# nv-tlabs/GEN3C

Hardware: NVIDIA H100
Metric: denoise-steps/sec, 7B DiT, 121-frame 720p latent (higher is better)
Workload: dtype bf16

## Files before the change

gen3c_b200/csrc/gemm_wgmma.cu:

```cuda
#include <cstdlib>
#include <cstring>

#include "kernels.h"

namespace g3c {

constexpr int BM = 128;
constexpr int BK = 64;
constexpr int WG_K = 16;
template <bool kFp8>
constexpr int kBlockK = kFp8 ? 2 * BK : BK;
constexpr int GEMM_THREADS = 384;

struct GemmParams {
  int M, N, K;
  int ldd;
  void* D;
  const float* gate;
  int num_m_blk, num_n_blk, num_k_blk;
  int super_n;
  const float* nr_gamma;
  const float* nr_cs;
  float nr_eps;
  const float* scale_a;
  const float* scale_b;
};

constexpr int EPI_NORM_ROPE_BF16 = 4;

template <int BN>
struct GemmSmem {
  static constexpr int kABytes = BM * BK * 2;
  static constexpr int kBBytes = BN * BK * 2;
  static constexpr int kStageBytes = kABytes + kBBytes;
  static constexpr int kStages = (192 * 1024) / kStageBytes;
  static constexpr int kBarBytes = 256;
  static constexpr int kTotal = kStages * kStageBytes + kBarBytes + 1024;
};

__device__ __forceinline__ float gelu_erf(float x) {
  return 0.5f * x * (1.0f + erff(x * 0.70710678118654752440f));
}

__device__ __forceinline__ void tile_coords(const GemmParams& p, int tile, int& m_blk, int& n_blk) {
  int per_super = p.num_m_blk * p.super_n;
  int sc = tile / per_super;
  int rem = tile - sc * per_super;
  int n0 = sc * p.super_n;
  int width = p.num_n_blk - n0 < p.super_n ? p.num_n_blk - n0 : p.super_n;
  m_blk = rem / width;
  n_blk = n0 + rem - m_blk * width;
}

template <int BN>
__device__ __forceinline__ void epilogue_norm_rope(const float (&acc)[BN / 2], const GemmParams& p, int row_a, int col_q,
                                                   int n_base) {
#pragma unroll
  for (int hd = 0; hd < BN / 128; ++hd) {
    if (n_base + hd * 128 >= p.N) break;
    float ss[2] = {0.f, 0.f};
#pragma unroll
    for (int i = 16 * hd; i < 16 * hd + 16; ++i) {
      ss[0] = fmaf(acc[4 * i], acc[4 * i], fmaf(acc[4 * i + 1], acc[4 * i + 1], ss[0]));
      ss[1] = fmaf(acc[4 * i + 2], acc[4 * i + 2], fmaf(acc[4 * i + 3], acc[4 * i + 3], ss[1]));
    }
#pragma unroll
    for (int h = 0; h < 2; ++h) {
      ss[h] += __shfl_xor_sync(0xffffffffu, ss[h], 1);
      ss[h] += __shfl_xor_sync(0xffffffffu, ss[h], 2);
    }
#pragma unroll
    for (int h = 0; h < 2; ++h) {
      const int row = row_a + 8 * h;
      if (row >= p.M) continue;
      const float rstd = rsqrtf(ss[h] * (1.0f / 128.0f) + p.nr_eps);
      const float* cs = p.nr_cs ? p.nr_cs + (size_t)row * 128 : nullptr;
      __nv_bfloat16* dptr = reinterpret_cast<__nv_bfloat16*>(p.D) + (size_t)row * p.ldd + n_base + hd * 128;
#pragma unroll
      for (int i = 0; i < 8; ++i) {
        const int c = 8 * i + col_q;
        const float2 ga = *reinterpret_cast<const float2*>(p.nr_gamma + c);
        const float2 gb = *reinterpret_cast<const float2*>(p.nr_gamma + 64 + c);
        const int ia = 4 * (16 * hd + i) + 2 * h, ib = 4 * (16 * hd + i + 8) + 2 * h;
        float a[2] = {acc[ia] * (rstd * ga.x), acc[ia + 1] * (rstd * ga.y)};
        float b[2] = {acc[ib] * (rstd * gb.x), acc[ib + 1] * (rstd * gb.y)};
        if (cs) {
          const float2 co = *reinterpret_cast<const float2*>(cs + c);
          const float2 si = *reinterpret_cast<const float2*>(cs + 64 + c);
          const float cv[2] = {co.x, co.y}, sv[2] = {si.x, si.y};
#pragma unroll
          for (int e = 0; e < 2; ++e) {
            const float n = a[e] * cv[e] - b[e] * sv[e], m = b[e] * cv[e] + a[e] * sv[e];
            a[e] = n;
            b[e] = m;
          }
        }
        *reinterpret_cast<uint32_t*>(dptr + c) = pack_bf16x2(a[0], a[1]);
        *reinterpret_cast<uint32_t*>(dptr + 64 + c) = pack_bf16x2(b[0], b[1]);
      }
    }
  }
}

template <int BN>
__device__ __forceinline__ void dequantise(float (&acc)[BN / 2], const GemmParams& p, int row_a, int col_q, int n_base) {
  float sa[2];
#pragma unroll
  for (int h = 0; h < 2; ++h) sa[h] = row_a + 8 * h < p.M ? p.scale_a[row_a + 8 * h] : 0.f;
#pragma unroll
  for (int i = 0; i < BN / 8; ++i) {
    const int col = n_base + 8 * i + col_q;
    float2 sb = make_float2(0.f, 0.f);
    if (col + 1 < p.N) sb = *reinterpret_cast<const float2*>(p.scale_b + col);
    else if (col < p.N) sb.x = p.scale_b[col];
#pragma unroll
    for (int h = 0; h < 2; ++h) {
      acc[4 * i + 2 * h] = acc[4 * i + 2 * h] * sa[h] * sb.x;
      acc[4 * i + 2 * h + 1] = acc[4 * i + 2 * h + 1] * sa[h] * sb.y;
    }
  }
}

template <int BN, int EPI>
__device__ __forceinline__ void epilogue(const float (&acc)[BN / 2], const GemmParams& p, int row_a, int col_q,
                                         int n_base) {
  if constexpr (EPI == EPI_NORM_ROPE_BF16) {
    epilogue_norm_rope<BN>(acc, p, row_a, col_q, n_base);
  } else {
#pragma unroll
    for (int h = 0; h < 2; ++h) {
      const int row = row_a + 8 * h;
      if (row >= p.M) continue;
#pragma unroll
      for (int i = 0; i < BN / 8; ++i) {
        const int col = n_base + 8 * i + col_q;
        if (col >= p.N) continue;
        const bool pair = col + 1 < p.N;
        float v0 = acc[4 * i + 2 * h], v1 = acc[4 * i + 2 * h + 1];
        if constexpr (EPI == G3C_EPI_BF16 || EPI == G3C_EPI_GELU_BF16) {
          if constexpr (EPI == G3C_EPI_GELU_BF16) {
            v0 = gelu_erf(v0);
            v1 = gelu_erf(v1);
          }
          __nv_bfloat16* dptr = reinterpret_cast<__nv_bfloat16*>(p.D) + (size_t)row * p.ldd + col;
          if (pair) *reinterpret_cast<uint32_t*>(dptr) = pack_bf16x2(v0, v1);
          else dptr[0] = __float2bfloat16_rn(v0);
        } else {
          float* dptr = reinterpret_cast<float*>(p.D) + (size_t)row * p.ldd + col;
          if constexpr (EPI == G3C_EPI_GATED_RESIDUAL_F32) {
            if (pair) {
              const float2 g = *reinterpret_cast<const float2*>(p.gate + col);
              float2 x = *reinterpret_cast<float2*>(dptr);
              x.x = fmaf(g.x, v0, x.x);
              x.y = fmaf(g.y, v1, x.y);
              *reinterpret_cast<float2*>(dptr) = x;
            } else {
              dptr[0] = fmaf(p.gate[col], v0, dptr[0]);
            }
          } else {
            if (pair) *reinterpret_cast<float2*>(dptr) = make_float2(v0, v1);
            else dptr[0] = v0;
          }
        }
      }
    }
  }
}

template <int BN, int EPI, bool kFp8>
__global__ void __launch_bounds__(GEMM_THREADS, 1)
    k_gemm(const __grid_constant__ CUtensorMap tmA, const __grid_constant__ CUtensorMap tmB, const GemmParams p) {
  using S = GemmSmem<BN>;
  constexpr int kStages = S::kStages;
  extern __shared__ uint8_t smem_raw[];
  uint8_t* smem = reinterpret_cast<uint8_t*>((reinterpret_cast<uintptr_t>(smem_raw) + 1023) &
                                             ~static_cast<uintptr_t>(1023));
  uint8_t* smem_a = smem;
  uint8_t* smem_b = smem + kStages * S::kABytes;
  uint64_t* bars = reinterpret_cast<uint64_t*>(smem + kStages * S::kStageBytes);
  uint64_t* full = bars;
  uint64_t* empty = bars + kStages;

  const uint32_t wg = threadIdx.x / 128;
  const uint32_t tid = threadIdx.x % 128;

  if (threadIdx.x == 0) {
    tma_prefetch_desc(&tmA);
    tma_prefetch_desc(&tmB);
    for (int i = 0; i < kStages; ++i) {
      mbar_init(&full[i], 1);
      mbar_init(&empty[i], 2);
    }
    fence_barrier_init();
  }
  __syncthreads();

  const int num_tiles = p.num_m_blk * p.num_n_blk;

  if (wg == 0) {
    setmaxnreg_dec<40>();
    if (tid == 0) {
      uint32_t stage = 0, phase = 0;
      for (int tile = blockIdx.x; tile < num_tiles; tile += gridDim.x) {
        int m_blk, n_blk;
        tile_coords(p, tile, m_blk, n_blk);
        for (int kb = 0; kb < p.num_k_blk; ++kb) {
          mbar_wait(&empty[stage], phase ^ 1);
          mbar_expect_tx(&full[stage], S::kStageBytes);
          tma_load_2d(smem_a + stage * S::kABytes, &tmA, &full[stage], kb * kBlockK<kFp8>, m_blk * BM);
          tma_load_2d(smem_b + stage * S::kBBytes, &tmB, &full[stage], kb * kBlockK<kFp8>, n_blk * BN);
          if (++stage == kStages) {
            stage = 0;
            phase ^= 1;
          }
        }
      }
    }
  } else {
    setmaxnreg_inc<232>();
    const uint32_t c = wg - 1;
    const uint32_t warp = tid / 32, lane = tid % 32;
    uint32_t stage = 0, phase = 0;
    float acc[BN / 2];
    for (int tile = blockIdx.x; tile < num_tiles; tile += gridDim.x) {
      int m_blk, n_blk;
      tile_coords(p, tile, m_blk, n_blk);
      if constexpr (kFp8) {
        static_assert(BN <= 128, "fp8 tiles hold two accumulator sets");
        float part[BN / 2];
#pragma unroll
        for (int i = 0; i < BN / 2; ++i) acc[i] = 0.f;
        for (int kb = 0; kb < p.num_k_blk; ++kb) {
          mbar_wait(&full[stage], phase);
          const uint64_t da = make_sdesc_sw128(smem_u32(smem_a + stage * S::kABytes + c * 64 * 128));
          const uint64_t db = make_sdesc_sw128(smem_u32(smem_b + stage * S::kBBytes));
          wgmma_fence();
#pragma unroll
          for (int k = 0; k < BK / WG_K; ++k) {
            const uint64_t a = sdesc_advance(da, k * WG_K * 2), b = sdesc_advance(db, k * WG_K * 2);
            if constexpr (BN == 128) wgmma_ss_n128_e4m3(part, a, b, k != 0 ? 1u : 0u);
            else wgmma_ss_n64_e4m3(part, a, b, k != 0 ? 1u : 0u);
          }
          wgmma_commit();
          wgmma_wait<0>();
          fence_regs(part);
          if (tid == 0) mbar_arrive(&empty[stage]);
#pragma unroll
          for (int i = 0; i < BN / 2; ++i) acc[i] += part[i];
          if (++stage == kStages) {
            stage = 0;
            phase ^= 1;
          }
        }
      } else {
        uint32_t prev_stage = 0;
        for (int kb = 0; kb < p.num_k_blk; ++kb) {
          mbar_wait(&full[stage], phase);
          const uint64_t da = make_sdesc_sw128(smem_u32(smem_a + stage * S::kABytes + c * 64 * 128));
          const uint64_t db = make_sdesc_sw128(smem_u32(smem_b + stage * S::kBBytes));
          wgmma_fence();
#pragma unroll
          for (int k = 0; k < BK / WG_K; ++k) {
            const uint64_t a = sdesc_advance(da, k * WG_K * 2), b = sdesc_advance(db, k * WG_K * 2);
            const uint32_t accumulate = (kb | k) != 0 ? 1u : 0u;
            if constexpr (BN == 256) wgmma_ss_n256(acc, a, b, accumulate);
            else if constexpr (BN == 128) wgmma_ss_n128(acc, a, b, accumulate);
            else wgmma_ss_n64(acc, a, b, accumulate);
          }
          wgmma_commit();
          wgmma_wait<1>();
          fence_regs(acc);
          if (kb > 0 && tid == 0) mbar_arrive(&empty[prev_stage]);
          prev_stage = stage;
          if (++stage == kStages) {
            stage = 0;
            phase ^= 1;
          }
        }
        wgmma_wait<0>();
        fence_regs(acc);
        if (tid == 0) mbar_arrive(&empty[prev_stage]);
      }
      const int row_a = m_blk * BM + (int)(c * 64 + warp * 16 + lane / 4), col_q = (int)(2 * (lane % 4));
      if constexpr (kFp8) dequantise<BN>(acc, p, row_a, col_q, n_blk * BN);
      epilogue<BN, EPI>(acc, p, row_a, col_q, n_blk * BN);
    }
  }
}

template <int BN, int EPI, bool kFp8>
static int launch_gemm(const CUtensorMap& tmA, const CUtensorMap& tmB, const GemmParams& p, cudaStream_t st) {
  using S = GemmSmem<BN>;
  static bool configured = false;
  if (!configured) {
    G3C_CUDA(cudaFuncSetAttribute(k_gemm<BN, EPI, kFp8>, cudaFuncAttributeMaxDynamicSharedMemorySize, S::kTotal));
    configured = true;
  }
  int tiles = p.num_m_blk * p.num_n_blk;
  int grid = tiles < sm_count() ? tiles : sm_count();
  k_gemm<BN, EPI, kFp8><<<grid, GEMM_THREADS, S::kTotal, st>>>(tmA, tmB, p);
  G3C_CUDA(cudaGetLastError());
  return G3C_OK;
}

template <int BN, bool kFp8>
static int dispatch_epi(int epi, const CUtensorMap& tmA, const CUtensorMap& tmB, const GemmParams& p, cudaStream_t st) {
  switch (epi) {
    case G3C_EPI_BF16: return launch_gemm<BN, G3C_EPI_BF16, kFp8>(tmA, tmB, p, st);
    case G3C_EPI_GELU_BF16: return launch_gemm<BN, G3C_EPI_GELU_BF16, kFp8>(tmA, tmB, p, st);
    case G3C_EPI_GATED_RESIDUAL_F32: return launch_gemm<BN, G3C_EPI_GATED_RESIDUAL_F32, kFp8>(tmA, tmB, p, st);
    case G3C_EPI_F32: return launch_gemm<BN, G3C_EPI_F32, kFp8>(tmA, tmB, p, st);
    case EPI_NORM_ROPE_BF16:
      if constexpr (BN >= 128) return launch_gemm<BN, EPI_NORM_ROPE_BF16, kFp8>(tmA, tmB, p, st);
      break;
  }
  set_error("gemm: unknown epilogue %d", epi);
  return G3C_EINVAL;
}

static int gemm_any(const void* A, const void* B, const float* scale_a, const float* scale_b, void* D, int M, int N,
                    int K, int lda, int ldb, int ldd, int epilogue, const float* gate, int block_n, cudaStream_t st,
                    const NormRope* norm_rope) {
  const bool fp8 = scale_a != nullptr;
  G3C_REQUIRE(A && B && D, "gemm: null operand");
  G3C_REQUIRE(epilogue >= G3C_EPI_BF16 && epilogue <= G3C_EPI_F32, "gemm: unknown epilogue %d", epilogue);
  if (norm_rope) {
    G3C_REQUIRE(epilogue == G3C_EPI_BF16 && N % 128 == 0 && norm_rope->gamma,
                "gemm: the RMSNorm/RoPE epilogue needs the bf16 epilogue, N %% 128 == 0 and a gain vector");
    G3C_REQUIRE((reinterpret_cast<uintptr_t>(norm_rope->gamma) & 15) == 0 &&
                    (reinterpret_cast<uintptr_t>(norm_rope->cs) & 15) == 0,
                "gemm: RMSNorm gain / RoPE table must be 16-byte aligned");
    epilogue = EPI_NORM_ROPE_BF16;
  }
  G3C_REQUIRE(M > 0 && N > 0 && K > 0, "gemm: bad shape %dx%dx%d", M, N, K);
  if (fp8)
    G3C_REQUIRE(K % 16 == 0 && lda % 16 == 0 && ldb % 16 == 0, "gemm_fp8: K/lda/ldb must be multiples of 16");
  else
    G3C_REQUIRE(K % 8 == 0 && lda % 8 == 0 && ldb % 8 == 0, "gemm: K/lda/ldb must be multiples of 8");
  G3C_REQUIRE(lda >= K && ldb >= K && ldd >= N, "gemm: leading dimension smaller than extent");
  if (epilogue == G3C_EPI_BF16 || epilogue == G3C_EPI_GELU_BF16 || epilogue == EPI_NORM_ROPE_BF16)
    G3C_REQUIRE(ldd % 8 == 0 && (reinterpret_cast<uintptr_t>(D) & 15) == 0,
                "gemm: bf16 output needs ldd %% 8 == 0 and 16-byte aligned base");
  else
    G3C_REQUIRE(ldd % 4 == 0 && (reinterpret_cast<uintptr_t>(D) & 15) == 0,
                "gemm: f32 output needs ldd %% 4 == 0 and 16-byte aligned base");
  G3C_REQUIRE(epilogue != G3C_EPI_GATED_RESIDUAL_F32 ||
                  (gate && (reinterpret_cast<uintptr_t>(gate) & 15) == 0),
              "gemm: gated-residual epilogue needs a 16-byte aligned gate vector");
  int bn = block_n;
  G3C_REQUIRE(bn == 0 || bn == 64 || bn == 128 || bn == 256 || bn == 512, "gemm: block_n %d unsupported", bn);
  if (bn == 512) {
    G3C_REQUIRE(N % 256 == 0, "gemm: block_n 512 needs N %% 256 == 0 (N=%d)", N);
    bn = 256;
  }
  if (bn == 0) bn = (N >= 256 && N % 256 == 0) ? 256 : (N > 64 ? 128 : 64);
  if (fp8 && bn == 256) bn = 128;
  G3C_REQUIRE(epilogue != EPI_NORM_ROPE_BF16 || bn >= 128, "gemm: the RMSNorm/RoPE epilogue needs tiles of whole heads");

  CUtensorMap tmA, tmB;
  const int esize = fp8 ? 1 : 2, bk = fp8 ? kBlockK<true> : kBlockK<false>;
  const CUtensorMapDataType dt = fp8 ? CU_TENSOR_MAP_DATA_TYPE_UINT8 : CU_TENSOR_MAP_DATA_TYPE_BFLOAT16;
  uint64_t dimsA[2] = {(uint64_t)K, (uint64_t)M}, strA[1] = {(uint64_t)lda * esize};
  uint32_t boxA[2] = {(uint32_t)bk, BM};
  int rc = make_tmap_bf16_sw128(&tmA, A, 2, dimsA, strA, boxA, dt);
  if (rc) return rc;
  uint64_t dimsB[2] = {(uint64_t)K, (uint64_t)N}, strB[1] = {(uint64_t)ldb * esize};
  uint32_t boxB[2] = {(uint32_t)bk, (uint32_t)bn};
  rc = make_tmap_bf16_sw128(&tmB, B, 2, dimsB, strB, boxB, dt);
  if (rc) return rc;

  GemmParams p;
  p.M = M;
  p.N = N;
  p.K = K;
  p.ldd = ldd;
  p.D = D;
  p.gate = gate;
  p.nr_gamma = norm_rope ? norm_rope->gamma : nullptr;
  p.nr_cs = norm_rope ? norm_rope->cs : nullptr;
  p.nr_eps = norm_rope ? norm_rope->eps : 0.0f;
  p.scale_a = scale_a;
  p.scale_b = scale_b;
  p.num_m_blk = (M + BM - 1) / BM;
  p.num_n_blk = (N + bn - 1) / bn;
  p.num_k_blk = (K + bk - 1) / bk;
  long long col_bytes = (long long)bn * K * esize;
  int sn = (int)((16ll << 20) / (col_bytes > 0 ? col_bytes : 1));
  if (sn < 1) sn = 1;
  if (sn > p.num_n_blk) sn = p.num_n_blk;
  p.super_n = sn;
  if (fp8) return bn == 64 ? dispatch_epi<64, true>(epilogue, tmA, tmB, p, st)
                           : dispatch_epi<128, true>(epilogue, tmA, tmB, p, st);
  switch (bn) {
    case 64: return dispatch_epi<64, false>(epilogue, tmA, tmB, p, st);
    case 128: return dispatch_epi<128, false>(epilogue, tmA, tmB, p, st);
    default: return dispatch_epi<256, false>(epilogue, tmA, tmB, p, st);
  }
}

int gemm_bf16(const void* A, const void* B, void* D, int M, int N, int K, int lda, int ldb, int ldd,
              int epilogue, const float* gate, int block_n, cudaStream_t st, const NormRope* norm_rope) {
  return gemm_any(A, B, nullptr, nullptr, D, M, N, K, lda, ldb, ldd, epilogue, gate, block_n, st, norm_rope);
}

int gemm_fp8(const void* A8, const float* scale_a, const void* B8, const float* scale_b, void* D, int M, int N, int K,
             int lda, int ldb, int ldd, int epilogue, const float* gate, int block_n, cudaStream_t st,
             const NormRope* norm_rope) {
  G3C_REQUIRE(scale_a && scale_b, "gemm_fp8: null scale vector");
  G3C_REQUIRE((reinterpret_cast<uintptr_t>(scale_a) & 15) == 0 && (reinterpret_cast<uintptr_t>(scale_b) & 15) == 0,
              "gemm_fp8: scale vectors must be 16-byte aligned");
  return gemm_any(A8, B8, scale_a, scale_b, D, M, N, K, lda, ldb, ldd, epilogue, gate, block_n, st, norm_rope);
}

}

extern "C" int g3c_gemm_bf16(const void* A, const void* B, void* D, int M, int N, int K, int lda,
                             int ldb, int ldd, int epilogue, const float* gate, int block_n,
                             void* stream) {
  return g3c::gemm_bf16(A, B, D, M, N, K, lda, ldb, ldd, epilogue, gate, block_n,
                        (cudaStream_t)stream);
}

extern "C" int g3c_gemm_fp8(const void* A8, const float* scale_A, const void* B8, const float* scale_B, void* D, int M,
                            int N, int K, int lda, int ldb, int ldd, int epilogue, const float* gate, int block_n,
                            void* stream) {
  return g3c::gemm_fp8(A8, scale_A, B8, scale_B, D, M, N, K, lda, ldb, ldd, epilogue, gate, block_n,
                       (cudaStream_t)stream);
}

extern "C" int g3c_gemm_norm_rope_fp8(const void* A8, const float* scale_A, const void* B8, const float* scale_B, void* D,
                                      int M, int N, int K, int lda, int ldb, int ldd, const float* gamma,
                                      const float* cos_sin, float eps, void* stream) {
  g3c::NormRope nr;
  nr.gamma = gamma;
  nr.cs = cos_sin;
  nr.eps = eps;
  return g3c::gemm_fp8(A8, scale_A, B8, scale_B, D, M, N, K, lda, ldb, ldd, G3C_EPI_BF16, nullptr, 0,
                       (cudaStream_t)stream, &nr);
}

extern "C" int g3c_gemm_norm_rope_bf16(const void* A, const void* B, void* D, int M, int N, int K, int lda, int ldb,
                                       int ldd, const float* gamma, const float* cos_sin, float eps, void* stream) {
  g3c::NormRope nr;
  nr.gamma = gamma;
  nr.cs = cos_sin;
  nr.eps = eps;
  return g3c::gemm_bf16(A, B, D, M, N, K, lda, ldb, ldd, G3C_EPI_BF16, nullptr, 0, (cudaStream_t)stream, &nr);
}
```

gen3c_b200/csrc/common.cuh:

```cuda
#pragma once
#include <cuda.h>
#include <cuda_bf16.h>
#include <cuda_runtime.h>
#include <stdint.h>
#include <stdio.h>

#include "../../include/gen3c_b200.h"
#include "wgmma_ops.cuh"

namespace g3c {

void set_error(const char* fmt, ...);
int cuda_fail(cudaError_t e, const char* what, const char* file, int line);
#define G3C_CUDA(x)                                                         \
  do {                                                                      \
    cudaError_t _e = (x);                                                   \
    if (_e != cudaSuccess) return ::g3c::cuda_fail(_e, #x, __FILE__, __LINE__); \
  } while (0)
#define G3C_REQUIRE(cond, ...)        \
  do {                                \
    if (!(cond)) {                    \
      ::g3c::set_error(__VA_ARGS__);  \
      return G3C_EINVAL;       \
    }                                 \
// ... 66 lines not shown
  return ok != 0;
}
__device__ __forceinline__ bool mbar_test(uint64_t* bar, uint32_t parity) {
  uint32_t ok;
  asm volatile(
      "{\n\t.reg .pred P;\n\t"
      "mbarrier.test_wait.parity.shared::cta.b64 P, [%1], %2;\n\t"
      "selp.b32 %0, 1, 0, P;\n\t}\n"
      : "=r"(ok)
      : "r"(smem_u32(bar)), "r"(parity)
      : "memory");
  return ok != 0;
}
#ifndef G3C_MBAR_TIMEOUT_NS
#define G3C_MBAR_TIMEOUT_NS 4000000000ull
#endif
__device__ __forceinline__ uint64_t global_timer_ns() {
  uint64_t t;
  asm volatile("mov.u64 %0, %%globaltimer;\n" : "=l"(t));
  return t;
}
#ifdef G3C_MBAR_DEBUG
#define G3C_MBAR_TIMEOUT_ACTION(bar, parity)                                                                 \
  do {                                                                                                       \
    printf("g3c: mbarrier timeout block(%d,%d) thread %d bar@%u parity %u\n", blockIdx.x, blockIdx.y,        \
           threadIdx.x, bar, parity);                                                                        \
    __trap();                                                                                                \
  } while (0)
#else
#define G3C_MBAR_TIMEOUT_ACTION(bar, parity) asm volatile("trap;\n")
#endif
__device__ __forceinline__ void mbar_wait(uint64_t* bar, uint32_t parity) {
  if (mbar_try_wait(bar, parity)) return;
  uint32_t spins = 0;
  uint64_t t0 = 0;
  while (!mbar_try_wait(bar, parity)) {
    if ((++spins & 0xFFFu) == 0) {
      uint64_t now = global_timer_ns();
      if (t0 == 0) t0 = now;
      else if (now - t0 > G3C_MBAR_TIMEOUT_NS) G3C_MBAR_TIMEOUT_ACTION(smem_u32(bar), parity);
    }
  }
}

__device__ __forceinline__ void mbar_wait_ns(uint64_t* bar, uint32_t parity, unsigned long long timeout_ns) {
  if (mbar_try_wait(bar, parity)) return;
  uint32_t spins = 0;
  uint64_t t0 = 0;
  while (!mbar_try_wait(bar, parity)) {
    if ((++spins & 0xFFFu) == 0) {
      uint64_t now = global_timer_ns();
      if (t0 == 0) t0 = now;
      else if (now - t0 > timeout_ns) G3C_MBAR_TIMEOUT_ACTION(smem_u32(bar), parity);
    }
  }
}

__device__ __forceinline__ void mbar_wait_ns_or_exit(uint64_t* bar, uint32_t parity, unsigned long long timeout_ns) {
  if (mbar_try_wait(bar, parity)) return;
  uint32_t spins = 0;
  uint64_t t0 = 0;
  while (!mbar_try_wait(bar, parity)) {
    if ((++spins & 0xFFFu) == 0) {
      uint64_t now = global_timer_ns();
      if (t0 == 0) t0 = now;
      else if (now - t0 > timeout_ns) asm volatile("exit;\n");
    }
  }
}

__device__ __forceinline__ bool bar_red_or(uint32_t id, uint32_t nthreads, bool pred) {
  uint32_t r;
  asm volatile(
      "{\n\t.reg .pred P, Q;\n\t"
      "setp.ne.u32 P, %1, 0;\n\t"
      "bar.red.or.pred Q, %2, %3, P;\n\t"
      "selp.u32 %0, 1, 0, Q;\n\t}\n"
      : "=r"(r)
      : "r"((uint32_t)pred), "r"(id), "r"(nthreads)
      : "memory");
  return r != 0;
}

__device__ __forceinline__ void tma_prefetch_desc(const CUtensorMap* m) {
  asm volatile("prefetch.tensormap [%0];\n" ::"l"(reinterpret_cast<uint64_t>(m)) : "memory");
}
__device__ __forceinline__ void tma_load_2d(void* smem_dst, const CUtensorMap* m, uint64_t* bar,
                                            int c0, int c1) {
  asm volatile(
      "cp.async.bulk.tensor.2d.shared::cluster.global.mbarrier::complete_tx::bytes"
      " [%0], [%1, {%3, %4}], [%2];\n" ::"r"(smem_u32(smem_dst)),
      "l"(reinterpret_cast<uint64_t>(m)), "r"(smem_u32(bar)), "r"(c0), "r"(c1)
      : "memory");
}
__device__ __forceinline__ void tma_load_3d(void* smem_dst, const CUtensorMap* m, uint64_t* bar,
                                            int c0, int c1, int c2) {
  asm volatile(
      "cp.async.bulk.tensor.3d.shared::cluster.global.mbarrier::complete_tx::bytes"
      " [%0], [%1, {%3, %4, %5}], [%2];\n" ::"r"(smem_u32(smem_dst)),
      "l"(reinterpret_cast<uint64_t>(m)), "r"(smem_u32(bar)), "r"(c0), "r"(c1), "r"(c2)
      : "memory");
}

__device__ __forceinline__ void tma_store_2d(const CUtensorMap* m, const void* smem_src, int c0, int c1) {
  asm volatile("cp.async.bulk.tensor.2d.global.shared::cta.bulk_group [%0, {%2, %3}], [%1];\n" ::"l"(
                   reinterpret_cast<uint64_t>(m)),
               "r"(smem_u32(smem_src)), "r"(c0), "r"(c1)
               : "memory");
}
__device__ __forceinline__ void tma_reduce_add_2d(const CUtensorMap* m, const void* smem_src, int c0, int c1) {
  asm volatile("cp.reduce.async.bulk.tensor.2d.global.shared::cta.add.bulk_group [%0, {%2, %3}], [%1];\n" ::"l"(
                   reinterpret_cast<uint64_t>(m)),
               "r"(smem_u32(smem_src)), "r"(c0), "r"(c1)
               : "memory");
}
__device__ __forceinline__ void tma_store_commit() { asm volatile("cp.async.bulk.commit_group;\n" ::: "memory"); }
template <int N>
__device__ __forceinline__ void tma_store_wait_read() {
  asm volatile("cp.async.bulk.wait_group.read %0;\n" ::"n"(N) : "memory");
}
template <int N>
__device__ __forceinline__ void tma_store_wait_all() {
  asm volatile("cp.async.bulk.wait_group %0;\n" ::"n"(N) : "memory");
}

__device__ __forceinline__ void wgmma_fence() { asm volatile("wgmma.fence.sync.aligned;\n" ::: "memory"); }
__device__ __forceinline__ void wgmma_commit() { asm volatile("wgmma.commit_group.sync.aligned;\n" ::: "memory"); }
template <int N>
__device__ __forceinline__ void wgmma_wait() {
  asm volatile("wgmma.wait_group.sync.aligned %0;\n" ::"n"(N) : "memory");
}
template <int N>
__device__ __forceinline__ void fence_regs(float (&r)[N]) {
#pragma unroll
  for (int i = 0; i < N; ++i) asm volatile("" : "+f"(r[i])::"memory");
}
template <int N>
__device__ __forceinline__ void fence_regs(uint32_t (&r)[N]) {
#pragma unroll
  for (int i = 0; i < N; ++i) asm volatile("" : "+r"(r[i])::"memory");
}

__device__ __forceinline__ uint64_t make_sdesc_sw128(uint32_t smem_addr) {
  uint64_t d = 0;
  d |= static_cast<uint64_t>((smem_addr & 0x3FFFFu) >> 4);
  d |= static_cast<uint64_t>(1) << 16;
  d |= static_cast<uint64_t>(1024u >> 4) << 32;
  d |= static_cast<uint64_t>(1) << 62;
  return d;
}
__device__ __forceinline__ uint64_t make_sdesc_sw128_mn(uint32_t smem_addr, uint32_t mn_block_bytes) {
  uint64_t d = 0;
  d |= static_cast<uint64_t>((smem_addr & 0x3FFFFu) >> 4);
  d |= static_cast<uint64_t>((mn_block_bytes >> 4) & 0x3FFFu) << 16;
  d |= static_cast<uint64_t>(1024u >> 4) << 32;
  d |= static_cast<uint64_t>(1) << 62;
  return d;
}
__device__ __forceinline__ uint64_t sdesc_advance(uint64_t d, uint32_t bytes) {
  return d + static_cast<uint64_t>(bytes >> 4);
}

template <int N>
__device__ __forceinline__ void setmaxnreg_dec() {
  asm volatile("setmaxnreg.dec.sync.aligned.u32 %0;\n" ::"n"(N));
}
// ... 23 lines not shown
```

Before: 0.1410.

## Vectorise GEMM epilogue stores via quad shuffles and batch gated-residual loads

The bf16 and norm+RoPE epilogues now swap packed values across each lane quad with shuffles, so every thread writes one 16-byte store instead of four 4-byte stores. Gamma for norm+RoPE is staged in shared memory and the cos/sin loads are hoisted out of the per-head loop. The gated-residual epilogue issues its gate and residual loads in batches before the FMAs and stores, giving more memory-level parallelism. The cost is extra shuffle instructions and higher register pressure in the epilogue.

```diff
diff --git a/gen3c_b200/csrc/gemm_wgmma.cu b/gen3c_b200/csrc/gemm_wgmma.cu
--- a/gen3c_b200/csrc/gemm_wgmma.cu
+++ b/gen3c_b200/csrc/gemm_wgmma.cu
@@ -35,7 +35,8 @@
   static constexpr int kStageBytes = kABytes + kBBytes;
   static constexpr int kStages = (192 * 1024) / kStageBytes;
   static constexpr int kBarBytes = 256;
-  static constexpr int kTotal = kStages * kStageBytes + kBarBytes + 1024;
+  static constexpr int kGammaBytes = 128 * 4;
+  static constexpr int kTotal = kStages * kStageBytes + kBarBytes + kGammaBytes + 1024;
 };
 
 __device__ __forceinline__ float gelu_erf(float x) {
@@ -52,51 +53,128 @@
   n_blk = n0 + rem - m_blk * width;
 }
 
+__device__ __forceinline__ uint4 quad_gather_bf16x8(const uint32_t (&v)[4]) {
+  const int lane = (int)(threadIdx.x % 32), q = lane % 4;
+  uint32_t w[4] = {0u, 0u, 0u, 0u};
+#pragma unroll
+  for (int r = 0; r < 4; ++r) {
+    const int js = (q + r) & 3, src = (q - r) & 3;
+    const uint32_t send = js == 0 ? v[0] : js == 1 ? v[1] : js == 2 ? v[2] : v[3];
+    const uint32_t got = r == 0 ? send : __shfl_sync(0xffffffffu, send, (lane & ~3) | src);
+#pragma unroll
+    for (int k = 0; k < 4; ++k) w[k] = src == k ? got : w[k];
+  }
+  return make_uint4(w[0], w[1], w[2], w[3]);
+}
+
 template <int BN>
-__device__ __forceinline__ void epilogue_norm_rope(const float (&acc)[BN / 2], const GemmParams& p, int row_a, int col_q,
-                                                   int n_base) {
-#pragma unroll
-  for (int hd = 0; hd < BN / 128; ++hd) {
-    if (n_base + hd * 128 >= p.N) break;
-    float ss[2] = {0.f, 0.f};
+__device__ __forceinline__ void epilogue_norm_rope(const float (&acc)[BN / 2], const GemmParams& p, const float* gamma_s,
+                                                   int row_a, int col_q, int n_base) {
+  constexpr int kHeads = BN / 128;
+  float ss[kHeads][2];
+#pragma unroll
+  for (int hd = 0; hd < kHeads; ++hd) {
+    ss[hd][0] = ss[hd][1] = 0.f;
 #pragma unroll
     for (int i = 16 * hd; i < 16 * hd + 16; ++i) {
-      ss[0] = fmaf(acc[4 * i], acc[4 * i], fmaf(acc[4 * i + 1], acc[4 * i + 1], ss[0]));
-      ss[1] = fmaf(acc[4 * i + 2], acc[4 * i + 2], fmaf(acc[4 * i + 3], acc[4 * i + 3], ss[1]));
+      ss[hd][0] = fmaf(acc[4 * i], acc[4 * i], fmaf(acc[4 * i + 1], acc[4 * i + 1], ss[hd][0]));
+      ss[hd][1] = fmaf(acc[4 * i + 2], acc[4 * i + 2], fmaf(acc[4 * i + 3], acc[4 * i + 3], ss[hd][1]));
     }
 #pragma unroll
     for (int h = 0; h < 2; ++h) {
-      ss[h] += __shfl_xor_sync(0xffffffffu, ss[h], 1);
-      ss[h] += __shfl_xor_sync(0xffffffffu, ss[h], 2);
-    }
-#pragma unroll
-    for (int h = 0; h < 2; ++h) {
-      const int row = row_a + 8 * h;
-      if (row >= p.M) continue;
-      const float rstd = rsqrtf(ss[h] * (1.0f / 128.0f) + p.nr_eps);
-      const float* cs = p.nr_cs ? p.nr_cs + (size_t)row * 128 : nullptr;
+      ss[hd][h] += __shfl_xor_sync(0xffffffffu, ss[hd][h], 1);
+      ss[hd][h] += __shfl_xor_sync(0xffffffffu, ss[hd][h], 2);
+    }
+  }
+#pragma unroll
+  for (int h = 0; h < 2; ++h) {
+    const int row = row_a + 8 * h;
+    const bool row_ok = row < p.M;
+    float2 co[8], si[8];
+    if (p.nr_cs && row_ok) {
+      const float* cs = p.nr_cs + (size_t)row * 128;
+#pragma unroll
+      for (int i = 0; i < 8; ++i) {
+        co[i] = *reinterpret_cast<const float2*>(cs + 8 * i + col_q);
+        si[i] = *reinterpret_cast<const float2*>(cs + 64 + 8 * i + col_q);
+      }
+    }
+#pragma unroll
+    for (int hd = 0; hd < kHeads; ++hd) {
+      if (n_base + hd * 128 >= p.N) break;
+      const float rstd = rsqrtf(ss[hd][h] * (1.0f / 128.0f) + p.nr_eps);
       __nv_bfloat16* dptr = reinterpret_cast<__nv_bfloat16*>(p.D) + (size_t)row * p.ldd + n_base + hd * 128;
 #pragma unroll
-      for (int i = 0; i < 8; ++i) {
-        const int c = 8 * i + col_q;
-        const float2 ga = *reinterpret_cast<const float2*>(p.nr_gamma + c);
-        const float2 gb = *reinterpret_cast<const float2*>(p.nr_gamma + 64 + c);
-        const int ia = 4 * (16 * hd + i) + 2 * h, ib = 4 * (16 * hd + i + 8) + 2 * h;
-        float a[2] = {acc[ia] * (rstd * ga.x), acc[ia + 1] * (rstd * ga.y)};
-        float b[2] = {acc[ib] * (rstd * gb.x), acc[ib + 1] * (rstd * gb.y)};
-        if (cs) {
-          const float2 co = *reinterpret_cast<const float2*>(cs + c);
-          const float2 si = *reinterpret_cast<const float2*>(cs + 64 + c);
-          const float cv[2] = {co.x, co.y}, sv[2] = {si.x, si.y};
-#pragma unroll
-          for (int e = 0; e < 2; ++e) {
-            const float n = a[e] * cv[e] - b[e] * sv[e], m = b[e] * cv[e] + a[e] * sv[e];
-            a[e] = n;
-            b[e] = m;
-          }
-        }
-        *reinterpret_cast<uint32_t*>(dptr + c) = pack_bf16x2(a[0], a[1]);
-        *reinterpret_cast<uint32_t*>(dptr + 64 + c) = pack_bf16x2(b[0], b[1]);
+      for (int i0 = 0; i0 < 8; i0 += 4) {
+        uint32_t pa[4], pb[4];
+#pragma unroll
+        for (int j = 0; j < 4; ++j) {
+          const int i = i0 + j, c = 8 * i + col_q;
+          const float2 ga = *reinterpret_cast<const float2*>(gamma_s + c);
+          const float2 gb = *reinterpret_cast<const float2*>(gamma_s + 64 + c);
+          const int ia = 4 * (16 * hd + i) + 2 * h, ib = 4 * (16 * hd + i + 8) + 2 * h;
+          float a[2] = {acc[ia] * (rstd * ga.x), acc[ia + 1] * (rstd * ga.y)};
+          float b[2] = {acc[ib] * (rstd * gb.x), acc[ib + 1] * (rstd * gb.y)};
+          if (p.nr_cs) {
+            const float cv[2] = {co[i].x, co[i].y}, sv[2] = {si[i].x, si[i].y};
+#pragma unroll
+            for (int e = 0; e < 2; ++e) {
+              const float n = a[e] * cv[e] - b[e] * sv[e], m = b[e] * cv[e] + a[e] * sv[e];
+              a[e] = n;
+              b[e] = m;
+            }
+          }
+          pa[j] = pack_bf16x2(a[0], a[1]);
+          pb[j] = pack_bf16x2(b[0], b[1]);
+        }
+        const uint4 wa = quad_gather_bf16x8(pa), wb = quad_gather_bf16x8(pb);
+        const int c16 = 8 * i0 + 4 * col_q;
+        if (row_ok) {
+          *reinterpret_cast<uint4*>(dptr + c16) = wa;
+          *reinterpret_cast<uint4*>(dptr + 64 + c16) = wb;
+        }
+      }
+    }
+  }
+}
+
+constexpr int kGatedBatch = 8;
+
+template <int BN>
+__device__ __forceinline__ void epilogue_gated(const float (&acc)[BN / 2], const GemmParams& p, int row_a, int col_q,
+                                               int n_base) {
+  constexpr int kB = BN / 8 < kGatedBatch ? BN / 8 : kGatedBatch;
+  float* const xbase = reinterpret_cast<float*>(p.D);
+#pragma unroll
+  for (int i0 = 0; i0 < BN / 8; i0 += kB) {
+    float2 g[kB], x[2][kB];
+#pragma unroll
+    for (int j = 0; j < kB; ++j) {
+      const int col = n_base + 8 * (i0 + j) + col_q;
+      if (col >= p.N) continue;
+      const bool pair = col + 1 < p.N;
+      g[j] = pair ? *reinterpret_cast<const float2*>(p.gate + col) : make_float2(p.gate[col], 0.f);
+#pragma unroll
+      for (int h = 0; h < 2; ++h) {
+        const int row = row_a + 8 * h;
+        if (row >= p.M) continue;
+        const float* xp = xbase + (size_t)row * p.ldd + col;
+        x[h][j] = pair ? *reinterpret_cast<const float2*>(xp) : make_float2(xp[0], 0.f);
+      }
+    }
+#pragma unroll
+    for (int j = 0; j < kB; ++j) {
+      const int i = i0 + j, col = n_base + 8 * i + col_q;
+      if (col >= p.N) continue;
+      const bool pair = col + 1 < p.N;
+#pragma unroll
+      for (int h = 0; h < 2; ++h) {
+        const int row = row_a + 8 * h;
+        if (row >= p.M) continue;
+        float* xp = xbase + (size_t)row * p.ldd + col;
+        const float v0 = acc[4 * i + 2 * h], v1 = acc[4 * i + 2 * h + 1];
+        if (pair) *reinterpret_cast<float2*>(xp) = make_float2(fmaf(g[j].x, v0, x[h][j].x), fmaf(g[j].y, v1, x[h][j].y));
+        else xp[0] = fmaf(g[j].x, v0, x[h][j].x);
       }
     }
   }
@@ -122,10 +200,33 @@
 }
 
 template <int BN, int EPI>
-__device__ __forceinline__ void epilogue(const float (&acc)[BN / 2], const GemmParams& p, int row_a, int col_q,
-                                         int n_base) {
+__device__ __forceinline__ void epilogue(const float (&acc)[BN / 2], const GemmParams& p, const float* gamma_s, int row_a,
+                                         int col_q, int n_base) {
   if constexpr (EPI == EPI_NORM_ROPE_BF16) {
-    epilogue_norm_rope<BN>(acc, p, row_a, col_q, n_base);
+    epilogue_norm_rope<BN>(acc, p, gamma_s, row_a, col_q, n_base);
+  } else if constexpr (EPI == G3C_EPI_GATED_RESIDUAL_F32) {
+    epilogue_gated<BN>(acc, p, row_a, col_q, n_base);
+  } else if ((EPI == G3C_EPI_BF16 || EPI == G3C_EPI_GELU_BF16) && n_base + BN <= p.N) {
+#pragma unroll
+    for (int h = 0; h < 2; ++h) {
+      const int row = row_a + 8 * h;
+      __nv_bfloat16* dptr = reinterpret_cast<__nv_bfloat16*>(p.D) + (size_t)row * p.ldd + n_base;
+#pragma unroll
+      for (int i0 = 0; i0 < BN / 8; i0 += 4) {
+        uint32_t v[4];
+#pragma unroll
+        for (int j = 0; j < 4; ++j) {
+          float v0 = acc[4 * (i0 + j) + 2 * h], v1 = acc[4 * (i0 + j) + 2 * h + 1];
+          if constexpr (EPI == G3C_EPI_GELU_BF16) {
+            v0 = gelu_erf(v0);
+            v1 = gelu_erf(v1);
+          }
+          v[j] = pack_bf16x2(v0, v1);
+        }
+        const uint4 w = quad_gather_bf16x8(v);
+        if (row < p.M) *reinterpret_cast<uint4*>(dptr + 8 * i0 + 4 * col_q) = w;
+      }
+    }
   } else {
 #pragma unroll
     for (int h = 0; h < 2; ++h) {
@@ -147,20 +248,8 @@
           else dptr[0] = __float2bfloat16_rn(v0);
         } else {
           float* dptr = reinterpret_cast<float*>(p.D) + (size_t)row * p.ldd + col;
-          if constexpr (EPI == G3C_EPI_GATED_RESIDUAL_F32) {
-            if (pair) {
-              const float2 g = *reinterpret_cast<const float2*>(p.gate + col);
-              float2 x = *reinterpret_cast<float2*>(dptr);
-              x.x = fmaf(g.x, v0, x.x);
-              x.y = fmaf(g.y, v1, x.y);
-              *reinterpret_cast<float2*>(dptr) = x;
-            } else {
-              dptr[0] = fmaf(p.gate[col], v0, dptr[0]);
-            }
-          } else {
-            if (pair) *reinterpret_cast<float2*>(dptr) = make_float2(v0, v1);
-            else dptr[0] = v0;
-          }
+          if (pair) *reinterpret_cast<float2*>(dptr) = make_float2(v0, v1);
+          else dptr[0] = v0;
         }
       }
     }
@@ -180,6 +269,7 @@
   uint64_t* bars = reinterpret_cast<uint64_t*>(smem + kStages * S::kStageBytes);
   uint64_t* full = bars;
   uint64_t* empty = bars + kStages;
+  float* gamma_s = reinterpret_cast<float*>(smem + kStages * S::kStageBytes + S::kBarBytes);
 
   const uint32_t wg = threadIdx.x / 128;
   const uint32_t tid = threadIdx.x % 128;
@@ -193,6 +283,8 @@
     }
     fence_barrier_init();
   }
+  if constexpr (EPI == EPI_NORM_ROPE_BF16)
+    if (threadIdx.x < 128) gamma_s[threadIdx.x] = p.nr_gamma[threadIdx.x];
   __syncthreads();
 
   const int num_tiles = p.num_m_blk * p.num_n_blk;
@@ -283,7 +375,7 @@
       }
       const int row_a = m_blk * BM + (int)(c * 64 + warp * 16 + lane / 4), col_q = (int)(2 * (lane % 4));
       if constexpr (kFp8) dequantise<BN>(acc, p, row_a, col_q, n_blk * BN);
-      epilogue<BN, EPI>(acc, p, row_a, col_q, n_blk * BN);
+      epilogue<BN, EPI>(acc, p, gamma_s, row_a, col_q, n_blk * BN);
     }
   }
 }
```

Result: faster. 0.1445 (median of 6 runs) (+2.4%).

## Stage GEMM epilogue through swizzled shared memory and store via TMA

Applied to the files above, without the earlier changes.

The GEMM epilogue now writes results into double-buffered, 128B-swizzled shared staging buffers per consumer warpgroup, then issues TMA bulk stores, or TMA reduce-add for the gated residual, instead of scattered per-thread global stores. A scalar path handles columns not covered by the 16-byte-aligned tensor map. The aim is coalesced, asynchronous output writes that overlap with the next tile's mainloop, and offloading the residual read-modify-write to TMA. In exchange it uses extra shared memory and adds named barriers and store-wait synchronisation per round. Read-only loads also switch to __ldg.

```diff
diff --git a/gen3c_b200/csrc/common.cuh b/gen3c_b200/csrc/common.cuh
--- a/gen3c_b200/csrc/common.cuh
+++ b/gen3c_b200/csrc/common.cuh
@@ -172,6 +172,10 @@
   return r != 0;
 }
 
+__device__ __forceinline__ void named_bar_sync(uint32_t id, uint32_t nthreads) {
+  asm volatile("bar.sync %0, %1;\n" ::"r"(id), "r"(nthreads) : "memory");
+}
+
 __device__ __forceinline__ void tma_prefetch_desc(const CUtensorMap* m) {
   asm volatile("prefetch.tensormap [%0];\n" ::"l"(reinterpret_cast<uint64_t>(m)) : "memory");
 }
diff --git a/gen3c_b200/csrc/gemm_wgmma.cu b/gen3c_b200/csrc/gemm_wgmma.cu
--- a/gen3c_b200/csrc/gemm_wgmma.cu
+++ b/gen3c_b200/csrc/gemm_wgmma.cu
@@ -15,6 +15,7 @@
 struct GemmParams {
   int M, N, K;
   int ldd;
+  int n_tma;
   void* D;
   const float* gate;
   int num_m_blk, num_n_blk, num_k_blk;
@@ -28,14 +29,21 @@
 
 constexpr int EPI_NORM_ROPE_BF16 = 4;
 
+constexpr int OUT_BOX_ROWS = 64;
+constexpr int OUT_BOX_BYTES = OUT_BOX_ROWS * 128;
+
 template <int BN>
 struct GemmSmem {
   static constexpr int kABytes = BM * BK * 2;
   static constexpr int kBBytes = BN * BK * 2;
   static constexpr int kStageBytes = kABytes + kBBytes;
   static constexpr int kStages = (192 * 1024) / kStageBytes;
+  static constexpr int kRingBytes = kStages * kStageBytes;
+  static constexpr int kStagingBytes = 2 * OUT_BOX_BYTES;
   static constexpr int kBarBytes = 256;
-  static constexpr int kTotal = kStages * kStageBytes + kBarBytes + 1024;
+  static constexpr int kTotal = kRingBytes + 2 * kStagingBytes + kBarBytes + 1024;
+  static_assert(kRingBytes % 1024 == 0, "the staging buffers need the 1024-byte alignment of the 128-byte swizzle");
+  static_assert(kTotal <= 227 * 1024, "shared memory per CTA");
 };
 
 __device__ __forceinline__ float gelu_erf(float x) {
@@ -52,9 +60,85 @@
   n_blk = n0 + rem - m_blk * width;
 }
 
+struct OutStage {
+  uint8_t* base;
+  uint32_t buf;
+  uint32_t bar_id;
+  bool leader;
+  uint32_t row;
+  uint32_t sw;
+  uint32_t col_q;
+};
+
+struct StageAddr {
+  uint32_t thr, sw16;
+};
+template <int kEsize>
+__device__ __forceinline__ StageAddr stage_addr_base(const OutStage& o) {
+  StageAddr a{o.buf + o.row + o.col_q * kEsize, o.sw << 4};
+  asm volatile("" : "+r"(a.thr), "+r"(a.sw16));
+  return a;
+}
+template <int kEsize>
+__device__ __forceinline__ uint32_t stage_addr(const StageAddr& a, int i, int h) {
+  constexpr int kGroupsPerBox = 128 / (8 * kEsize);
+  const uint32_t col_byte = (uint32_t)(i % kGroupsPerBox) * 8 * kEsize;
+  const uint32_t box = (uint32_t)(i / kGroupsPerBox) % 2;
+  return ((a.thr + h * 8 * 128 + col_byte) ^ a.sw16) + box * OUT_BOX_BYTES;
+}
+__device__ __forceinline__ void st_shared_b32(uint32_t addr, uint32_t v) {
+  asm volatile("st.shared.b32 [%0], %1;\n" ::"r"(addr), "r"(v));
+}
+__device__ __forceinline__ void st_shared_f32x2(uint32_t addr, float a, float b) {
+  asm volatile("st.shared.v2.f32 [%0], {%1, %2};\n" ::"r"(addr), "f"(a), "f"(b));
+}
+__device__ __forceinline__ void stage_acquire(const OutStage& o) {
+  if (o.leader) tma_store_wait_read<0>();
+  named_bar_sync(o.bar_id, 128);
+}
+template <bool kReduce, int kEsize>
+__device__ __forceinline__ void stage_issue(const OutStage& o, const CUtensorMap* tmD, int nbox, int box_cols, int col0,
+                                            int row0, const GemmParams& p) {
+  fence_proxy_async();
+  named_bar_sync(o.bar_id, 128);
+  if (p.n_tma < p.N && p.n_tma >= col0 && p.n_tma < col0 + nbox * box_cols) {
+    const int ntail = p.N - p.n_tma, tid = (int)(threadIdx.x % 128);
+#pragma unroll 1
+    for (int e = tid; e < OUT_BOX_ROWS * ntail; e += 128) {
+      const int r = e / ntail, col = p.n_tma + e % ntail;
+      if (row0 + r >= p.M) break;
+      const uint32_t byte = (uint32_t)((col - col0) % box_cols) * kEsize;
+      const uint32_t off = (uint32_t)((col - col0) / box_cols) * OUT_BOX_BYTES + r * 128 +
+                           ((((byte >> 4) ^ (uint32_t)(r % 8))) << 4) + (byte & 15);
+      const size_t g = (size_t)(row0 + r) * p.ldd + col;
+      uint32_t v;
+      if constexpr (kEsize == 2) {
+        asm volatile("ld.shared.u16 %0, [%1];\n" : "=r"(v) : "r"(o.buf + off));
+        reinterpret_cast<uint16_t*>(p.D)[g] = (uint16_t)v;
+      } else {
+        asm volatile("ld.shared.b32 %0, [%1];\n" : "=r"(v) : "r"(o.buf + off));
+        float* d = reinterpret_cast<float*>(p.D) + g;
+        *d = kReduce ? *d + __uint_as_float(v) : __uint_as_float(v);
+      }
+    }
+  }
+  if (o.leader && row0 < p.M) {
+    for (int b = 0; b < nbox; ++b) {
+      if (col0 + b * box_cols >= p.n_tma) break;
+      if constexpr (kReduce) tma_reduce_add_2d(tmD, o.base + b * OUT_BOX_BYTES, col0 + b * box_cols, row0);
+      else tma_store_2d(tmD, o.base + b * OUT_BOX_BYTES, col0 + b * box_cols, row0);
+    }
+    tma_store_commit();
+  }
+}
+
 template <int BN>
-__device__ __forceinline__ void epilogue_norm_rope(const float (&acc)[BN / 2], const GemmParams& p, int row_a, int col_q,
+__device__ __forceinline__ void epilogue_norm_rope(const float (&acc)[BN / 2], const GemmParams& p,
+                                                   const CUtensorMap* tmD, const OutStage& o, int row_a, int row0,
                                                    int n_base) {
+  const float* __restrict__ gamma = p.nr_gamma;
+  const float* __restrict__ cs_tab = p.nr_cs;
+  const int col_q = (int)o.col_q;
 #pragma unroll
   for (int hd = 0; hd < BN / 128; ++hd) {
     if (n_base + hd * 128 >= p.N) break;
@@ -69,24 +153,25 @@
       ss[h] += __shfl_xor_sync(0xffffffffu, ss[h], 1);
       ss[h] += __shfl_xor_sync(0xffffffffu, ss[h], 2);
     }
+    stage_acquire(o);
+    const StageAddr sa = stage_addr_base<2>(o);
 #pragma unroll
     for (int h = 0; h < 2; ++h) {
       const int row = row_a + 8 * h;
       if (row >= p.M) continue;
       const float rstd = rsqrtf(ss[h] * (1.0f / 128.0f) + p.nr_eps);
-      const float* cs = p.nr_cs ? p.nr_cs + (size_t)row * 128 : nullptr;
-      __nv_bfloat16* dptr = reinterpret_cast<__nv_bfloat16*>(p.D) + (size_t)row * p.ldd + n_base + hd * 128;
+      const float* cs = cs_tab ? cs_tab + (size_t)row * 128 : nullptr;
 #pragma unroll
       for (int i = 0; i < 8; ++i) {
         const int c = 8 * i + col_q;
-        const float2 ga = *reinterpret_cast<const float2*>(p.nr_gamma + c);
-        const float2 gb = *reinterpret_cast<const float2*>(p.nr_gamma + 64 + c);
+        const float2 ga = __ldg(reinterpret_cast<const float2*>(gamma + c));
+        const float2 gb = __ldg(reinterpret_cast<const float2*>(gamma + 64 + c));
         const int ia = 4 * (16 * hd + i) + 2 * h, ib = 4 * (16 * hd + i + 8) + 2 * h;
         float a[2] = {acc[ia] * (rstd * ga.x), acc[ia + 1] * (rstd * ga.y)};
         float b[2] = {acc[ib] * (rstd * gb.x), acc[ib + 1] * (rstd * gb.y)};
         if (cs) {
-          const float2 co = *reinterpret_cast<const float2*>(cs + c);
-          const float2 si = *reinterpret_cast<const float2*>(cs + 64 + c);
+          const float2 co = __ldg(reinterpret_cast<const float2*>(cs + c));
+          const float2 si = __ldg(reinterpret_cast<const float2*>(cs + 64 + c));
           const float cv[2] = {co.x, co.y}, sv[2] = {si.x, si.y};
 #pragma unroll
           for (int e = 0; e < 2; ++e) {
@@ -95,24 +180,27 @@
             b[e] = m;
           }
         }
-        *reinterpret_cast<uint32_t*>(dptr + c) = pack_bf16x2(a[0], a[1]);
-        *reinterpret_cast<uint32_t*>(dptr + 64 + c) = pack_bf16x2(b[0], b[1]);
+        st_shared_b32(stage_addr<2>(sa, i, h), pack_bf16x2(a[0], a[1]));
+        st_shared_b32(stage_addr<2>(sa, i + 8, h), pack_bf16x2(b[0], b[1]));
       }
     }
+    stage_issue<false, 2>(o, tmD, 2, 64, n_base + hd * 128, row0, p);
   }
 }
 
 template <int BN>
 __device__ __forceinline__ void dequantise(float (&acc)[BN / 2], const GemmParams& p, int row_a, int col_q, int n_base) {
+  const float* __restrict__ scale_a = p.scale_a;
+  const float* __restrict__ scale_b = p.scale_b;
   float sa[2];
 #pragma unroll
-  for (int h = 0; h < 2; ++h) sa[h] = row_a + 8 * h < p.M ? p.scale_a[row_a + 8 * h] : 0.f;
+  for (int h = 0; h < 2; ++h) sa[h] = row_a + 8 * h < p.M ? __ldg(scale_a + row_a + 8 * h) : 0.f;
 #pragma unroll
   for (int i = 0; i < BN / 8; ++i) {
     const int col = n_base + 8 * i + col_q;
     float2 sb = make_float2(0.f, 0.f);
-    if (col + 1 < p.N) sb = *reinterpret_cast<const float2*>(p.scale_b + col);
-    else if (col < p.N) sb.x = p.scale_b[col];
+    if (col + 1 < p.N) sb = __ldg(reinterpret_cast<const float2*>(scale_b + col));
+    else if (col < p.N) sb.x = __ldg(scale_b + col);
 #pragma unroll
     for (int h = 0; h < 2; ++h) {
       acc[4 * i + 2 * h] = acc[4 * i + 2 * h] * sa[h] * sb.x;
@@ -122,54 +210,54 @@
 }
 
 template <int BN, int EPI>
-__device__ __forceinline__ void epilogue(const float (&acc)[BN / 2], const GemmParams& p, int row_a, int col_q,
-                                         int n_base) {
-  if constexpr (EPI == EPI_NORM_ROPE_BF16) {
-    epilogue_norm_rope<BN>(acc, p, row_a, col_q, n_base);
-  } else {
-#pragma unroll
-    for (int h = 0; h < 2; ++h) {
-      const int row = row_a + 8 * h;
-      if (row >= p.M) continue;
-#pragma unroll
-      for (int i = 0; i < BN / 8; ++i) {
-        const int col = n_base + 8 * i + col_q;
-        if (col >= p.N) continue;
-        const bool pair = col + 1 < p.N;
+__device__ __forceinline__ void epilogue(const float (&acc)[BN / 2], const GemmParams& p, const CUtensorMap* tmD,
+                                         const OutStage& o, int row0, int n_base) {
+  constexpr bool kGated = EPI == G3C_EPI_GATED_RESIDUAL_F32;
+  constexpr int kEsize = (kGated || EPI == G3C_EPI_F32) ? 4 : 2;
+  constexpr int kBoxCols = 128 / kEsize;
+  constexpr int kRoundGroups = 2 * kBoxCols / 8 < BN / 8 ? 2 * kBoxCols / 8 : BN / 8;
+  constexpr int kRoundBoxes = (8 * kRoundGroups + kBoxCols - 1) / kBoxCols;
+  const float* __restrict__ gate = p.gate;
+#pragma unroll
+  for (int rd = 0; rd < BN / 8 / kRoundGroups; ++rd) {
+    float2 g[kGated ? kRoundGroups : 1];
+    if constexpr (kGated) {
+#pragma unroll
+      for (int j = 0; j < kRoundGroups; ++j) {
+        const int col = n_base + 8 * (rd * kRoundGroups + j) + (int)o.col_q;
+        g[j] = make_float2(0.f, 0.f);
+        if (col + 1 < p.N) g[j] = __ldg(reinterpret_cast<const float2*>(gate + col));
+        else if (col < p.N) g[j].x = __ldg(gate + col);
+      }
+    }
+    stage_acquire(o);
+    const StageAddr sa = stage_addr_base<kEsize>(o);
+#pragma unroll
+    for (int j = 0; j < kRoundGroups; ++j) {
+      const int i = rd * kRoundGroups + j;
+#pragma unroll
+      for (int h = 0; h < 2; ++h) {
         float v0 = acc[4 * i + 2 * h], v1 = acc[4 * i + 2 * h + 1];
-        if constexpr (EPI == G3C_EPI_BF16 || EPI == G3C_EPI_GELU_BF16) {
-          if constexpr (EPI == G3C_EPI_GELU_BF16) {
-            v0 = gelu_erf(v0);
-            v1 = gelu_erf(v1);
-          }
-          __nv_bfloat16* dptr = reinterpret_cast<__nv_bfloat16*>(p.D) + (size_t)row * p.ldd + col;
-          if (pair) *reinterpret_cast<uint32_t*>(dptr) = pack_bf16x2(v0, v1);
-          else dptr[0] = __float2bfloat16_rn(v0);
-        } else {
-          float* dptr = reinterpret_cast<float*>(p.D) + (size_t)row * p.ldd + col;
-          if constexpr (EPI == G3C_EPI_GATED_RESIDUAL_F32) {
-            if (pair) {
-              const float2 g = *reinterpret_cast<const float2*>(p.gate + col);
-              float2 x = *reinterpret_cast<float2*>(dptr);
-              x.x = fmaf(g.x, v0, x.x);
-              x.y = fmaf(g.y, v1, x.y);
-              *reinterpret_cast<float2*>(dptr) = x;
-            } else {
-              dptr[0] = fmaf(p.gate[col], v0, dptr[0]);
-            }
-          } else {
-            if (pair) *reinterpret_cast<float2*>(dptr) = make_float2(v0, v1);
-            else dptr[0] = v0;
-          }
+        if constexpr (EPI == G3C_EPI_GELU_BF16) {
+          v0 = gelu_erf(v0);
+          v1 = gelu_erf(v1);
         }
+        if constexpr (kGated) {
+          v0 = g[j].x * v0;
+          v1 = g[j].y * v1;
+        }
+        if constexpr (kEsize == 2) st_shared_b32(stage_addr<2>(sa, i, h), pack_bf16x2(v0, v1));
+        else st_shared_f32x2(stage_addr<4>(sa, i, h), v0, v1);
       }
     }
+    stage_issue<kGated, kEsize>(o, tmD, kRoundBoxes, kBoxCols, n_base + rd * 8 * kRoundGroups, row0, p);
   }
 }
 
 template <int BN, int EPI, bool kFp8>
 __global__ void __launch_bounds__(GEMM_THREADS, 1)
-    k_gemm(const __grid_constant__ CUtensorMap tmA, const __grid_constant__ CUtensorMap tmB, const GemmParams p) {
+    k_gemm(const __grid_constant__ CUtensorMap tmA, const __grid_constant__ CUtensorMap tmB,
+           const __grid_constant__ CUtensorMap tmD, const GemmParams p) {
   using S = GemmSmem<BN>;
   constexpr int kStages = S::kStages;
   extern __shared__ uint8_t smem_raw[];
@@ -177,7 +265,8 @@
                                              ~static_cast<uintptr_t>(1023));
   uint8_t* smem_a = smem;
   uint8_t* smem_b = smem + kStages * S::kABytes;
-  uint64_t* bars = reinterpret_cast<uint64_t*>(smem + kStages * S::kStageBytes);
+  uint8_t* staging = smem + S::kRingBytes;
+  uint64_t* bars = reinterpret_cast<uint64_t*>(staging + 2 * S::kStagingBytes);
   uint64_t* full = bars;
   uint64_t* empty = bars + kStages;
 
@@ -187,6 +276,7 @@
   if (threadIdx.x == 0) {
     tma_prefetch_desc(&tmA);
     tma_prefetch_desc(&tmB);
+    tma_prefetch_desc(&tmD);
     for (int i = 0; i < kStages; ++i) {
       mbar_init(&full[i], 1);
       mbar_init(&empty[i], 2);
@@ -220,6 +310,14 @@
     setmaxnreg_inc<232>();
     const uint32_t c = wg - 1;
     const uint32_t warp = tid / 32, lane = tid % 32;
+    OutStage out;
+    out.base = staging + c * S::kStagingBytes;
+    out.buf = smem_u32(out.base);
+    out.bar_id = 1 + c;
+    out.leader = tid == 0;
+    out.row = (16 * warp + lane / 4) * 128;
+    out.sw = lane / 4;
+    out.col_q = 2 * (lane % 4);
     uint32_t stage = 0, phase = 0;
     float acc[BN / 2];
     for (int tile = blockIdx.x; tile < num_tiles; tile += gridDim.x) {
@@ -281,15 +379,18 @@
         fence_regs(acc);
         if (tid == 0) mbar_arrive(&empty[prev_stage]);
       }
-      const int row_a = m_blk * BM + (int)(c * 64 + warp * 16 + lane / 4), col_q = (int)(2 * (lane % 4));
-      if constexpr (kFp8) dequantise<BN>(acc, p, row_a, col_q, n_blk * BN);
-      epilogue<BN, EPI>(acc, p, row_a, col_q, n_blk * BN);
-    }
+      const int row0 = m_blk * BM + (int)c * 64, row_a = row0 + (int)(warp * 16 + lane / 4);
+      if constexpr (kFp8) dequantise<BN>(acc, p, row_a, (int)out.col_q, n_blk * BN);
+      if constexpr (EPI == EPI_NORM_ROPE_BF16) epilogue_norm_rope<BN>(acc, p, &tmD, out, row_a, row0, n_blk * BN);
+      else epilogue<BN, EPI>(acc, p, &tmD, out, row0, n_blk * BN);
+    }
+    if (out.leader) tma_store_wait_all<0>();
   }
 }
 
 template <int BN, int EPI, bool kFp8>
-static int launch_gemm(const CUtensorMap& tmA, const CUtensorMap& tmB, const GemmParams& p, cudaStream_t st) {
+static int launch_gemm(const CUtensorMap& tmA, const CUtensorMap& tmB, const CUtensorMap& tmD, const GemmParams& p,
+                       cudaStream_t st) {
   using S = GemmSmem<BN>;
   static bool configured = false;
   if (!configured) {
@@ -298,20 +399,21 @@
   }
   int tiles = p.num_m_blk * p.num_n_blk;
   int grid = tiles < sm_count() ? tiles : sm_count();
-  k_gemm<BN, EPI, kFp8><<<grid, GEMM_THREADS, S::kTotal, st>>>(tmA, tmB, p);
+  k_gemm<BN, EPI, kFp8><<<grid, GEMM_THREADS, S::kTotal, st>>>(tmA, tmB, tmD, p);
   G3C_CUDA(cudaGetLastError());
   return G3C_OK;
 }
 
 template <int BN, bool kFp8>
-static int dispatch_epi(int epi, const CUtensorMap& tmA, const CUtensorMap& tmB, const GemmParams& p, cudaStream_t st) {
+static int dispatch_epi(int epi, const CUtensorMap& tmA, const CUtensorMap& tmB, const CUtensorMap& tmD,
+                        const GemmParams& p, cudaStream_t st) {
   switch (epi) {
-    case G3C_EPI_BF16: return launch_gemm<BN, G3C_EPI_BF16, kFp8>(tmA, tmB, p, st);
-    case G3C_EPI_GELU_BF16: return launch_gemm<BN, G3C_EPI_GELU_BF16, kFp8>(tmA, tmB, p, st);
-    case G3C_EPI_GATED_RESIDUAL_F32: return launch_gemm<BN, G3C_EPI_GATED_RESIDUAL_F32, kFp8>(tmA, tmB, p, st);
-    case G3C_EPI_F32: return launch_gemm<BN, G3C_EPI_F32, kFp8>(tmA, tmB, p, st);
+    case G3C_EPI_BF16: return launch_gemm<BN, G3C_EPI_BF16, kFp8>(tmA, tmB, tmD, p, st);
+    case G3C_EPI_GELU_BF16: return launch_gemm<BN, G3C_EPI_GELU_BF16, kFp8>(tmA, tmB, tmD, p, st);
+    case G3C_EPI_GATED_RESIDUAL_F32: return launch_gemm<BN, G3C_EPI_GATED_RESIDUAL_F32, kFp8>(tmA, tmB, tmD, p, st);
+    case G3C_EPI_F32: return launch_gemm<BN, G3C_EPI_F32, kFp8>(tmA, tmB, tmD, p, st);
     case EPI_NORM_ROPE_BF16:
-      if constexpr (BN >= 128) return launch_gemm<BN, EPI_NORM_ROPE_BF16, kFp8>(tmA, tmB, p, st);
+      if constexpr (BN >= 128) return launch_gemm<BN, EPI_NORM_ROPE_BF16, kFp8>(tmA, tmB, tmD, p, st);
       break;
   }
   set_error("gemm: unknown epilogue %d", epi);
@@ -357,7 +459,7 @@
   if (fp8 && bn == 256) bn = 128;
   G3C_REQUIRE(epilogue != EPI_NORM_ROPE_BF16 || bn >= 128, "gemm: the RMSNorm/RoPE epilogue needs tiles of whole heads");
 
-  CUtensorMap tmA, tmB;
+  CUtensorMap tmA, tmB, tmD;
   const int esize = fp8 ? 1 : 2, bk = fp8 ? kBlockK<true> : kBlockK<false>;
   const CUtensorMapDataType dt = fp8 ? CU_TENSOR_MAP_DATA_TYPE_UINT8 : CU_TENSOR_MAP_DATA_TYPE_BFLOAT16;
   uint64_t dimsA[2] = {(uint64_t)K, (uint64_t)M}, strA[1] = {(uint64_t)lda * esize};
@@ -368,12 +470,21 @@
   uint32_t boxB[2] = {(uint32_t)bk, (uint32_t)bn};
   rc = make_tmap_bf16_sw128(&tmB, B, 2, dimsB, strB, boxB, dt);
   if (rc) return rc;
+  const bool f32_out = epilogue == G3C_EPI_GATED_RESIDUAL_F32 || epilogue == G3C_EPI_F32;
+  const int dsize = f32_out ? 4 : 2;
+  const int n_tma = N / (16 / dsize) * (16 / dsize);
+  uint64_t dimsD[2] = {(uint64_t)(n_tma > 0 ? n_tma : 16 / dsize), (uint64_t)M}, strD[1] = {(uint64_t)ldd * dsize};
+  uint32_t boxD[2] = {(uint32_t)(128 / dsize), (uint32_t)OUT_BOX_ROWS};
+  rc = make_tmap_bf16_sw128(&tmD, D, 2, dimsD, strD, boxD,
+                            f32_out ? CU_TENSOR_MAP_DATA_TYPE_FLOAT32 : CU_TENSOR_MAP_DATA_TYPE_BFLOAT16);
+  if (rc) return rc;
 
   GemmParams p;
   p.M = M;
   p.N = N;
   p.K = K;
   p.ldd = ldd;
+  p.n_tma = n_tma;
   p.D = D;
   p.gate = gate;
   p.nr_gamma = norm_rope ? norm_rope->gamma : nullptr;
@@ -389,12 +500,12 @@
   if (sn < 1) sn = 1;
   if (sn > p.num_n_blk) sn = p.num_n_blk;
   p.super_n = sn;
-  if (fp8) return bn == 64 ? dispatch_epi<64, true>(epilogue, tmA, tmB, p, st)
-                           : dispatch_epi<128, true>(epilogue, tmA, tmB, p, st);
+  if (fp8) return bn == 64 ? dispatch_epi<64, true>(epilogue, tmA, tmB, tmD, p, st)
+                           : dispatch_epi<128, true>(epilogue, tmA, tmB, tmD, p, st);
   switch (bn) {
-    case 64: return dispatch_epi<64, false>(epilogue, tmA, tmB, p, st);
-    case 128: return dispatch_epi<128, false>(epilogue, tmA, tmB, p, st);
-    default: return dispatch_epi<256, false>(epilogue, tmA, tmB, p, st);
+    case 64: return dispatch_epi<64, false>(epilogue, tmA, tmB, tmD, p, st);
+    case 128: return dispatch_epi<128, false>(epilogue, tmA, tmB, tmD, p, st);
+    default: return dispatch_epi<256, false>(epilogue, tmA, tmB, tmD, p, st);
   }
 }
 
```

Measured after the change: 0.1414 before, 0.1473 after (median of 6 runs). +4.1%, better.
